# ScottHCL/recommend

Measured on AMD Instinct MI355X. Metric: ranked samples/sec (fwd+bwd) at B=4096 seq=128; AUC parity vs ref, higher is better.
Workload: dtype f32-emulated (fp16-pair / split-bf16); 1 GPU; C2: OneTrans 4L d128 H4 f512 L_NS12 L_S128 (seq 3x42), Criteo-shape 13 dense + 26 ids, replicated tables, fwd+bwd+optimizer; global_batch=4096, per_gpu_batch=4096, seq_len=128, parallelism=dp1

## Files before the change

### include/onetrans_hip.h

```cpp
#ifndef ONETRANS_HIP_H
#define ONETRANS_HIP_H

#include <stddef.h>
#include <stdint.h>

#ifdef __cplusplus
extern "C" {
#endif

#define OT_OK 0
#define OT_ERR_INVALID_ARG 1
#define OT_ERR_UNSUPPORTED 2
#define OT_ERR_HIP 3

#define OT_GEMM_NN 0
#define OT_GEMM_NT 1

#define OT_AX_NONE 0
#define OT_AX_RMSNORM 1
#define OT_AX_GELU 2
#define OT_AX_BF16 4
#define OT_AX_BF16_RMSNORM 5

#define OT_EPI_BIAS 1
// ... 9 lines not shown
#define OT_EPI_AUX_BF16 1024
#define OT_WG_D_BF16 8
#define OT_WG_D_KEEPBITS 16

int ot_version(void);
const char* ot_get_last_error_string(void);

int ot_gemm_tile_rows(void);
#define OT_MATMUL_F32 0
#define OT_MATMUL_SPLIT_BF16 1
#define OT_MATMUL_BF16 2
int ot_mixed_gemm(int mode, const float* A, int64_t lda, int K, const int32_t* in_rows,
                  int a_xform, const float* a_rstd, const float* a_gamma,
                  const float* W, int64_t w_gstride, int64_t ldw, int N,
                  const int32_t* tile_group, int ntiles,
                  const float* bias, int64_t bias_gstride,
                  float* C, int64_t ldc, const int32_t* out_rows, int epi,
                  const float* res, int64_t ldres, int res_tok,
                  const float* aux, int64_t ldaux,
                  uint32_t seed, uint32_t site, float drop_rate, int tail_K, int tail_I,
                  const int32_t* tail_pos, int precision, void* stream);
typedef struct ot_rms_epilogue {
  size_t struct_size;
  float* rstd_out; float eps;
  const float* x; int64_t ldx;
  const float* gamma; const float* rstd;
  const float* dres; int64_t lddres;
  int dres_tail_K, dres_tail_I;
  const int32_t* dres_tail_inv;
  float* dx_masked; int64_t lddxm;
  float* dgamma; int accumulate_dgamma;
  void* workspace; size_t ws_bytes;
  float* rowdot; int rowdot_n;
  uint16_t* gelu_out; int64_t ldgelu;
  uint16_t* xn_out; int64_t ldxn;
  uint16_t* c16_out; int64_t ldc16;
  float* rowmax_out; int rowmax_n;
  const float* a_rowmax; int a_rowmax_n;
  float* amax_out;
  float* rowabs_out; int rowabs_n;
} ot_rms_epilogue;
size_t ot_mixed_gemm_rms_workspace_size(int ntiles, int N);
int ot_mixed_gemm_rms(int mode, const float* A, int64_t lda, int K, const int32_t* in_rows,
                      int a_xform, const float* a_rstd, const float* a_gamma,
                      const float* W, int64_t w_gstride, int64_t ldw, int N,
                      const int32_t* tile_group, int ntiles,
                      const float* bias, int64_t bias_gstride,
                      float* C, int64_t ldc, const int32_t* out_rows, int epi,
                      const float* res, int64_t ldres, int res_tok,
                      const float* aux, int64_t ldaux,
                      uint32_t seed, uint32_t site, float drop_rate, int tail_K, int tail_I,
                      const int32_t* tail_pos, const ot_rms_epilogue* rms, int precision, void* stream);

size_t ot_wgrad_workspace_size(int nchunks, int K, int N);
int ot_mixed_gemm_wgrad(const float* A, int64_t lda, const int32_t* a_rows, int a_xform,
                        const float* a_rstd, const float* a_gamma,
                        const float* D, int64_t ldd, const int32_t* d_rows, int K, int N,
                        const int32_t* chunks, int nchunks, const int32_t* gchunk, int ngroups,
                        float* dW, int64_t dw_gstride, float* db, int64_t db_gstride,
                        int accumulate, void* workspace, size_t ws_bytes, int precision, void* stream);

int ot_mixed_gemm_wgrad_ex(const float* A, int64_t lda, const int32_t* a_rows, int a_xform,
                           const float* a_rstd, const float* a_gamma,
                           const float* D, int64_t ldd, const int32_t* d_rows, int K, int N,
                           const int32_t* chunks, int nchunks, const int32_t* gchunk, int ngroups,
                           float* dW, int64_t dw_gstride, float* db, int64_t db_gstride,
                           int accumulate, void* workspace, size_t ws_bytes, const float* a_bound,
                           const float* d_bound, int precision, void* stream);

int ot_mixed_gemm_wgrad_keep(const float* A, int64_t lda, const int32_t* a_rows, int a_xform,
                             const float* D, int64_t ldd, const int32_t* d_rows, int K, int N,
                             const int32_t* chunks, int nchunks, const int32_t* gchunk, int ngroups,
                             float* dW, int64_t dw_gstride, float* db, int64_t db_gstride,
                             int accumulate, void* workspace, size_t ws_bytes, const float* a_bound,
                             const float* d_bound, const uint32_t* keep, int64_t ldkeep, float d_scale,
                             int precision, void* stream);

int ot_transpose_banks(const float* src, float* dst, const int64_t* banks_dev, int nbanks, int64_t total_tiles,
                       void* stream);

size_t ot_split_image_elems(int G, int N, int K);
int ot_split_images(const float* base, const int64_t* desc_dev, int ndesc, int64_t total_units, uint16_t* img,
                    int precision, void* stream);
int ot_mixed_gemm_img(int mode, const float* A, int64_t lda, int K, const int32_t* in_rows,
                      int a_xform, const float* a_rstd, const float* a_gamma,
                      const float* W, int64_t w_gstride, int64_t ldw, int N,
                      const int32_t* tile_group, int ntiles,
                      const float* bias, int64_t bias_gstride,
                      float* C, int64_t ldc, const int32_t* out_rows, int epi,
                      const float* res, int64_t ldres, int res_tok,
                      const float* aux, int64_t ldaux,
                      uint32_t seed, uint32_t site, float drop_rate, int tail_K, int tail_I,
                      const int32_t* tail_pos, const uint16_t* b_image, int image_ntn, int image_tn0,
                      int precision, void* stream);
int ot_plane_wide(int on);
int ot_wgrad_wide(int on);
int ot_plane_rowmeta(int on);
int ot_plane_panel(int on);
int ot_plane_panel_launches(void);
int ot_mixed_gemm_rms_img(int mode, const float* A, int64_t lda, int K, const int32_t* in_rows,
                          int a_xform, const float* a_rstd, const float* a_gamma,
                          const float* W, int64_t w_gstride, int64_t ldw, int N,
                          const int32_t* tile_group, int ntiles,
                          const float* bias, int64_t bias_gstride,
                          float* C, int64_t ldc, const int32_t* out_rows, int epi,
                          const float* res, int64_t ldres, int res_tok,
                          const float* aux, int64_t ldaux,
                          uint32_t seed, uint32_t site, float drop_rate, int tail_K, int tail_I,
                          const int32_t* tail_pos, const ot_rms_epilogue* rms, const uint16_t* b_image,
                          int image_ntn, int image_tn0, int precision, void* stream);

typedef struct ot_ffn_fused_args {
  size_t struct_size;
  const float* x1; int64_t ldx1;
  const int32_t* rows;
  const int32_t* tile_group; int ntiles;
  const float* rstd;
  const uint16_t* w1_image; int w1_groups;
  const uint16_t* w2_image; int w2_groups;
  const float* b1; int64_t b1_gstride;
  const float* b2; int64_t b2_gstride;
  int f;
  float* u_out; int64_t ldu;
  float* u_amax;
  float* x2; int64_t ldx2;
  float* rstd_out; float eps;
  uint32_t seed, site; float drop_rate;
  int tail_K, tail_I; const int32_t* tail_pos;
} ot_ffn_fused_args;
int ot_ffn_fused_fwd(const ot_ffn_fused_args* args, void* stream);
int ot_ffn_fused(int on);

typedef struct ot_ffn_fused_bwd_args {
  size_t struct_size;
  const float* dy2; int64_t lddy2;
  const float* dy2_rowmax; int dy2_rowmax_n;
  const int32_t* rows;
  const int32_t* tile_group; int ntiles;
  const uint16_t* w2_image; int w2_groups;
  const uint16_t* w1_image; int w1_groups;
  int f;
  const float* u; int64_t ldu;
  float* du; int64_t lddu;
  float* du_amax;
  const float* x1; int64_t ldx1;
  const float* gamma; const float* rstd;
  const float* dres; int64_t lddres;
  float* dx1; int64_t lddx1;
  float* dx_masked; int64_t lddxm;
  float* dgamma; int accumulate_dgamma;
  void* workspace; size_t ws_bytes;
  float* amax_out; float* rowabs_out; int rowabs_n;
  uint32_t seed, site; float drop_rate;
  int tail_K, tail_I; const int32_t* tail_pos;
} ot_ffn_fused_bwd_args;
int ot_ffn_fused_bwd(const ot_ffn_fused_bwd_args* args, void* stream);
int ot_ffn_fused_bwd_on(int on);
int ot_ffn_fused_bwd_mask(const ot_ffn_fused_bwd_args* args, uint32_t mask_site, uint32_t* keep_out, int64_t ldkeep,
                          void* stream);
int ot_bwd_mask_fused(int on);

int ot_attn_fwd(const float* qkv, int64_t ld, int B, int H, int I, int K, const int32_t* qpos,
                int head_dim, float* out, float* lse, int precision, void* stream);
size_t ot_attn_fwd_fp8_workspace_size(int B, int H, int I, int head_dim);
int ot_attn_fwd_fp8(const float* qkv, int64_t ld, int B, int H, int I, int K, const int32_t* qpos,
                    int head_dim, float* out, float* lse, void* workspace, size_t ws_bytes, void* stream);
// ... 274 lines not shown
```

### recommend_amd/_lib.py

```python

from __future__ import annotations

import ctypes
import os
from ctypes import c_float, c_int, c_int64, c_size_t, c_uint32, c_void_p, c_char_p

_HERE = os.path.dirname(os.path.abspath(__file__))
LIB_PATH = os.environ.get('ONETRANS_HIP_LIB') or os.path.join(_HERE, 'libonetrans_hip.so')
HEADER = os.path.join(os.path.dirname(_HERE), 'include', 'onetrans_hip.h')

OT_GEMM_NN, OT_GEMM_NT = 0, 1
OT_AX_NONE, OT_AX_RMSNORM, OT_AX_GELU, OT_AX_BF16, OT_AX_BF16_RMSNORM = 0, 1, 2, 4, 5
OT_EPI_BIAS, OT_EPI_GELU_BWD, OT_EPI_GELU = 1, 2, 4
OT_EPI_DROPOUT, OT_EPI_RESIDUAL, OT_EPI_ACCUMULATE = 8, 16, 32
OT_EPI_ROW_RSTD, OT_EPI_RMSNORM_BWD, OT_EPI_ROWDOT = 64, 128, 256
OT_EPI_C_BF16 = 512
OT_EPI_AUX_BF16 = 1024
OT_ATTN_DQKV_BF16 = 1
OT_ATTN_QKV_BF16 = 2
OT_ATTN_DQ_PART_BF16 = 4
OT_WG_D_BF16 = 8
OT_WG_D_KEEPBITS = 16
OT_MATMUL_F32, OT_MATMUL_SPLIT_BF16, OT_MATMUL_BF16 = 0, 1, 2
OT_FP8_DEQUANT, OT_FP8_TWO_TERM = 1, 2
# ... 28 lines not shown
                ('tile_group', c_void_p), ('ntiles', c_int), ('rstd', c_void_p),
                ('w1_image', c_void_p), ('w1_groups', c_int), ('w2_image', c_void_p), ('w2_groups', c_int),
                ('b1', c_void_p), ('b1_gstride', c_int64), ('b2', c_void_p), ('b2_gstride', c_int64),
                ('f', c_int), ('u_out', c_void_p), ('ldu', c_int64), ('u_amax', c_void_p),
                ('x2', c_void_p), ('ldx2', c_int64), ('rstd_out', c_void_p), ('eps', c_float),
                ('seed', c_uint32), ('site', c_uint32), ('drop_rate', c_float),
                ('tail_K', c_int), ('tail_I', c_int), ('tail_pos', c_void_p)]


class FfnFusedBwdArgs(ctypes.Structure):
    _fields_ = [('struct_size', c_size_t), ('dy2', c_void_p), ('lddy2', c_int64),
                ('dy2_rowmax', c_void_p), ('dy2_rowmax_n', c_int), ('rows', c_void_p),
                ('tile_group', c_void_p), ('ntiles', c_int),
                ('w2_image', c_void_p), ('w2_groups', c_int), ('w1_image', c_void_p), ('w1_groups', c_int),
                ('f', c_int), ('u', c_void_p), ('ldu', c_int64), ('du', c_void_p), ('lddu', c_int64),
                ('du_amax', c_void_p), ('x1', c_void_p), ('ldx1', c_int64), ('gamma', c_void_p), ('rstd', c_void_p),
                ('dres', c_void_p), ('lddres', c_int64), ('dx1', c_void_p), ('lddx1', c_int64),
                ('dx_masked', c_void_p), ('lddxm', c_int64), ('dgamma', c_void_p), ('accumulate_dgamma', c_int),
                ('workspace', c_void_p), ('ws_bytes', c_size_t),
                ('amax_out', c_void_p), ('rowabs_out', c_void_p), ('rowabs_n', c_int),
                ('seed', c_uint32), ('site', c_uint32), ('drop_rate', c_float),
                ('tail_K', c_int), ('tail_I', c_int), ('tail_pos', c_void_p)]


class SeqTime(ctypes.Structure):
    _fields_ = [('times', c_void_p), ('stride_b', c_int64), ('L', ctypes.c_int32), ('map_off', ctypes.c_int32)]


class NsBag(ctypes.Structure):
    _fields_ = [('table', c_void_p), ('ids', c_void_p), ('weights', c_void_p), ('row_offset', c_int64),
                ('num_rows', c_int64), ('ids_stride', c_int64), ('weights_stride', c_int64),
                ('width', ctypes.c_int32), ('cap', ctypes.c_int32), ('col', ctypes.c_int32),
                ('pooling', ctypes.c_int32)]


OT_BAG_SUM, OT_BAG_MEAN = 0, 1
BAG_POOLINGS = {'sum': OT_BAG_SUM, 'mean': OT_BAG_MEAN}
NS_BAG_MAX = 32
NS_BAG_MAX_WIDTH = 256
SEQ_TIME_MAX_L = 4096
SEQ_TIME_MAX_SEQ = 32

P = c_void_p
I64 = c_int64

SIGNATURES = {
    'ot_version': (c_int, []),
    'ot_get_last_error_string': (c_char_p, []),
    'ot_gemm_tile_rows': (c_int, []),
    'ot_mixed_gemm': (c_int, [c_int, P, I64, c_int, P, c_int, P, P, P, I64, I64, c_int, P, c_int, P, I64,
                              P, I64, P, c_int, P, I64, c_int, P, I64, c_uint32, c_uint32, c_float, c_int,
                              c_int, P, c_int, P]),
    'ot_mixed_gemm_rms_workspace_size': (c_size_t, [c_int, c_int]),
    'ot_mixed_gemm_rms': (c_int, [c_int, P, I64, c_int, P, c_int, P, P, P, I64, I64, c_int, P, c_int, P, I64,
                                  P, I64, P, c_int, P, I64, c_int, P, I64, c_uint32, c_uint32, c_float, c_int,
                                  c_int, P, P, c_int, P]),
    'ot_wgrad_workspace_size': (c_size_t, [c_int, c_int, c_int]),
    'ot_mixed_gemm_wgrad': (c_int, [P, I64, P, c_int, P, P, P, I64, P, c_int, c_int, P, c_int, P, c_int, P,
                                    I64, P, I64, c_int, P, c_size_t, c_int, P]),
    'ot_mixed_gemm_wgrad_ex': (c_int, [P, I64, P, c_int, P, P, P, I64, P, c_int, c_int, P, c_int, P, c_int, P,
                                       I64, P, I64, c_int, P, c_size_t, P, P, c_int, P]),
    'ot_mixed_gemm_wgrad_keep': (c_int, [P, I64, P, c_int, P, I64, P, c_int, c_int, P, c_int, P, c_int, P, I64, P,
                                         I64, c_int, P, c_size_t, P, P, P, I64, c_float, c_int, P]),
    'ot_transpose_banks': (c_int, [P, P, P, c_int, I64, P]),
    'ot_mixed_gemm_img': (c_int, [c_int, P, I64, c_int, P, c_int, P, P, P, I64, I64, c_int, P, c_int, P, I64,
                                  P, I64, P, c_int, P, I64, c_int, P, I64, c_uint32, c_uint32, c_float, c_int,
                                  c_int, P, P, c_int, c_int, c_int, P]),
    'ot_mixed_gemm_rms_img': (c_int, [c_int, P, I64, c_int, P, c_int, P, P, P, I64, I64, c_int, P, c_int, P, I64,
                                      P, I64, P, c_int, P, I64, c_int, P, I64, c_uint32, c_uint32, c_float, c_int,
                                      c_int, P, P, P, c_int, c_int, c_int, P]),
    'ot_split_image_elems': (c_size_t, [c_int, c_int, c_int]),
    'ot_plane_wide': (c_int, [c_int]),
    'ot_wgrad_wide': (c_int, [c_int]),
    'ot_plane_rowmeta': (c_int, [c_int]),
    'ot_plane_panel': (c_int, [c_int]),
    'ot_plane_panel_launches': (c_int, []),
    'ot_ffn_fused_fwd': (c_int, [P, P]),
    'ot_ffn_fused': (c_int, [c_int]),
    'ot_ffn_fused_bwd': (c_int, [P, P]),
    'ot_ffn_fused_bwd_on': (c_int, [c_int]),
    'ot_ffn_fused_bwd_mask': (c_int, [P, c_uint32, P, I64, P]),
    'ot_bwd_mask_fused': (c_int, [c_int]),
    'ot_split_images': (c_int, [P, P, c_int, I64, P, c_int, P]),
    'ot_attn_fwd': (c_int, [P, I64, c_int, c_int, c_int, c_int, P, c_int, P, P, c_int, P]),
    'ot_attn_fwd_fp8_workspace_size': (c_size_t, [c_int, c_int, c_int, c_int]),
    'ot_attn_fwd_fp8': (c_int, [P, I64, c_int, c_int, c_int, c_int, P, c_int, P, P, P, c_size_t, P]),
    'ot_attn_fwd_fp8_ex': (c_int, [P, I64, c_int, c_int, c_int, c_int, P, c_int, P, P, P, c_size_t, c_int, P]),
    'ot_attn_fwd_fp8_deq16': (c_int, [P, I64, c_int, c_int, c_int, c_int, P, c_int, P, P, P, c_size_t, c_int, P, P]),
    'ot_attn_bwd_workspace_size': (c_size_t, [c_int, c_int, c_int]),
    'ot_attn_bwd': (c_int, [P, I64, P, P, P, c_int, c_int, c_int, c_int, P, c_int, P, P, c_int, P]),
    'ot_attn_bwd_ex_workspace_size': (c_size_t, [c_int, c_int, c_int, c_int, c_int, c_int, c_int]),
    'ot_attn_bwd_ex': (c_int, [P, I64, P, P, P, c_int, c_int, c_int, c_int, P, c_int, P, P, c_size_t, c_int, P]),
    'ot_attn_bwd_dqkv_bf16_supported': (c_int, [c_int, c_int, c_int, c_int, c_int]),
    'ot_attn_bwd_bf16_forms': (c_int, [c_int, c_int, c_int, c_int, c_int]),
    'ot_attn_slice_supported': (c_int, [c_int, c_int, c_int, c_int]),
    'ot_attn_bwd_flags_workspace_size': (c_size_t, [c_int, c_int, c_int, c_int, c_int, c_int, c_int, c_int]),
    'ot_attn_bwd_flags': (c_int, [P, I64, P, P, P, c_int, c_int, c_int, c_int, P, c_int, P, c_int, P, c_size_t, c_int, P]),
    'ot_attn_fwd_cached': (c_int, [P, I64, P, I64, P, c_int, c_int, c_int, c_int, c_int, c_int, P, P]),
    'ot_attn_fwd_cached_lse': (c_int, [P, I64, P, I64, P, c_int, c_int, c_int, c_int, c_int, c_int, P, P, P]),
    'ot_attn_bwd_cached_workspace_size': (c_size_t, [c_int, c_int, c_int, c_int, c_int, c_int, c_int]),
    'ot_attn_bwd_cached': (c_int, [P, I64, P, I64, P, c_int, c_int, c_int, c_int, c_int, c_int, c_int, P, P, P, P, P,
                                   c_int, P, c_size_t, P]),
    'ot_attn_amax_supported': (c_int, [c_int, c_int, c_int, c_int, c_int]),
    'ot_attn_fwd_amax': (c_int, [P, I64, c_int, c_int, c_int, c_int, P, c_int, P, P, P, P, c_int, P]),
    'ot_attn_bwd_amax': (c_int, [P, I64, P, P, P, c_int, c_int, c_int, c_int, P, c_int, P, P, c_size_t, P, P, c_int,
                                 P]),
    'ot_pyramid_select': (c_int, [P, c_float, c_int, c_int, c_int, c_int, P, P, P, c_int, P]),
    'ot_rmsnorm_fwd': (c_int, [P, I64, P, P, I64, P, I64, c_int, c_float, P]),
    'ot_rmsnorm_bwd_workspace_size': (c_size_t, [I64, c_int]),
    'ot_rmsnorm_bwd': (c_int, [P, I64, P, I64, P, P, P, I64, c_int, c_int, P, P, I64, P, I64, c_uint32,
                               c_uint32, c_float, c_int, c_int, P, P, c_int, I64, c_int, P, c_size_t, P]),
    'ot_dropout_apply': (c_int, [P, I64, P, I64, I64, c_int, c_uint32, c_uint32, c_float, c_int, c_int, P, P]),
    'ot_dropout_apply_bf16': (c_int, [P, I64, P, I64, I64, c_int, c_uint32, c_uint32, c_float, c_int, c_int, P, P]),
    'ot_rows_absmax': (c_int, [P, I64, I64, c_int, P, c_int, P]),
    'ot_dropout_rowmax_supported': (c_int, [c_int]),
    'ot_dropout_apply_ex': (c_int, [P, I64, P, I64, I64, c_int, c_uint32, c_uint32, c_float, c_int, c_int, P, P, P,
                                    c_int, P]),
    'ot_rows_colsum_workspace_size': (c_size_t, [I64, c_int]),
    'ot_rows_colsum': (c_int, [P, I64, P, I64, c_int, P, c_int, P, c_size_t, P]),
    'ot_ns_assemble': (c_int, [P, c_int, P, c_int, P, I64, P]),
    'ot_ns_grad_pack': (c_int, [P, c_int, c_int, P, I64, c_int, P, P, P]),
    'ot_fill_rows': (c_int, [P, I64, P, I64, P, c_int, P]),
    'ot_seq_rows': (c_int, [P, I64, c_int, c_int, I64, P, P]),
    'ot_head_fwd': (c_int, [P, P, P, c_int, c_int, c_int, P, P, P]),
    'ot_head_bwd_workspace_size': (c_size_t, [c_int, c_int, c_int]),
    'ot_head_bwd': (c_int, [P, P, P, P, c_int, c_int, c_int, P, P, P, I64, I64, c_int, P, c_size_t, P]),
    'ot_bce_workspace_size': (c_size_t, [c_int, c_int]),
    'ot_bce_fwd': (c_int, [P, P, c_int, c_int, P, P, c_size_t, P]),
    'ot_bce_bwd': (c_int, [P, P, P, c_int, c_int, P, P]),
    'ot_task_loss_fwd': (c_int, [P, P, c_int, c_int, c_uint32, P, P, c_size_t, P]),
    'ot_task_loss_bwd': (c_int, [P, P, P, c_int, c_int, c_uint32, P, P]),
    'ot_task_loss_logits_fwd': (c_int, [P, P, P, c_int, c_int, c_uint32, P, P, c_size_t, P]),
    'ot_task_loss_logits_bwd': (c_int, [P, P, P, c_int, c_int, c_uint32, P, P]),
    'ot_task_loss_weighted_workspace_size': (c_size_t, [c_int, c_int]),
    'ot_task_loss_weighted_fwd': (c_int, [P, P, P, P, I64, P, c_int, c_int, c_uint32, c_int, P, P, P, c_size_t, P]),
    'ot_task_loss_weighted_bwd': (c_int, [P, P, P, I64, P, P, P, c_int, c_int, c_uint32, c_int, P, P]),
    'ot_head_bwd_ex': (c_int, [P, P, P, P, P, c_int, c_int, c_int, P, P, P, I64, I64, c_int, P, c_size_t, P]),
    'ot_sparse_adagrad_workspace_size': (c_size_t, [I64, c_int]),
    'ot_sparse_adagrad': (c_int, [P, P, c_int, I64, P, P, I64, c_float, c_float, c_float, P, c_size_t, P]),
    'ot_sparse_grad_dense': (c_int, [c_int, I64, P, P, I64, P, P, c_size_t, P]),
    'ot_dense_adagrad_workspace_size': (c_size_t, []),
    'ot_dense_adagrad': (c_int, [P, P, P, I64, c_int, c_float, c_float, c_float, P, c_size_t, P]),
    'ot_sparse_prepare': (c_int, [c_int, I64, P, P, I64, P, P, c_size_t, P]),
    'ot_sparse_finish': (c_int, [P, P, c_int, I64, c_float, c_float, c_float, P, P, c_size_t, P]),
    'ot_sparse_adagrad_rowwise': (c_int, [P, P, c_int, I64, P, P, I64, c_float, c_float, c_float, P, c_size_t, P]),
    'ot_dense_adagrad_rowwise': (c_int, [P, P, P, I64, c_int, c_float, c_float, c_float, P, c_size_t, P]),
    'ot_sparse_finish_rowwise': (c_int, [P, P, c_int, I64, c_float, c_float, c_float, P, P, c_size_t, P]),
    'ot_shard_route_workspace_size': (c_size_t, [I64]),
    'ot_shard_route': (c_int, [P, I64, I64, c_int, P, P, P, P, c_size_t, P]),
    'ot_shard_route_unique_workspace_size': (c_size_t, [I64]),
    'ot_shard_route_unique': (c_int, [P, I64, I64, c_int, P, P, P, P, P, P, c_size_t, P]),
    'ot_segment_rows_sum': (c_int, [P, P, P, I64, c_int, P, P]),
    'ot_segment_rows_sum_workspace_size': (c_size_t, [I64, I64, c_int]),
    'ot_segment_rows_sum_ex': (c_int, [P, P, P, I64, I64, c_int, P, P, c_size_t, P]),
    'ot_gather_rows': (c_int, [P, c_int, P, I64, P, P]),
    'ot_permute_rows': (c_int, [P, P, I64, c_int, c_int, P, P]),
    'ot_hash_uniform_rows': (c_int, [P, I64, c_int, c_int, c_int, c_uint32, c_float, c_float, P]),
    'ot_clip_rmsprop_workspace_size': (c_size_t, [c_int, I64]),
    'ot_clip_rmsprop': (c_int, [P, P, P, P, P, c_int, I64, c_float, c_float, c_float, c_float, c_float, P,
                                c_size_t, P]),
    'ot_clip_adam_workspace_size': (c_size_t, [c_int, I64]),
    'ot_clip_adam': (c_int, [P, P, P, P, P, c_int, I64, c_float, c_float, c_float, c_float, I64, c_float, P,
                             c_size_t, P]),
    'ot_metrics_workspace_size': (c_size_t, [c_int, c_int]),
    'ot_metrics_update': (c_int, [P, P, c_int, c_int, I64, P, c_int, P, P, P, c_size_t, P]),
    'ot_metrics_weighted_workspace_size': (c_size_t, [c_int, c_int]),
# ... 78 lines not shown
```

### recommend_amd/csrc/gemm_images.hip

```cpp
#include "gemm.h"

namespace ot {

__device__ __forceinline__ const int64_t* image_unit(const int64_t* desc, int nd, int64_t unit, int64_t& g, int64_t& tn,
                                                     int64_t& ks) {
  int b = 0;
  while (b + 1 < nd && desc[10 * (b + 1) + 6] <= unit) ++b;
  const int64_t* d = desc + 10 * b;
  const int64_t G = d[7], N = d[8], K = d[9];
  const int64_t ntn = (N + GT - 1) / GT, nks = K / 16;
  int64_t u = unit - d[6];
  if (u >= G * ntn * nks) return nullptr;
  g = u / (ntn * nks);
  u %= ntn * nks;
  tn = u / nks;
  ks = u % nks;
  return d;
}

__global__ __launch_bounds__(256) void image_colscale_kernel(const float* __restrict__ base, const int64_t* __restrict__ desc,
                                                             int nd, uint16_t* img) {
  int64_t g, tn, ks;
  const int64_t* d = image_unit(desc, nd, blockIdx.x, g, tn, ks);
  if (!d || ks != 0 || d[4] == -1) return;
  const int64_t N = d[8], K = d[9];
  const int n = threadIdx.x >> 1, hh = threadIdx.x & 1;
  const int64_t gn = tn * GT + n;
  float m = 0.f;
  if (gn < N) {
    const float* src = base + d[0] + g * d[3] + gn * d[1];
#pragma unroll 8
    for (int64_t k = hh; k < K; k += 2) {
      float x = src[k * d[2]];
      if (d[4] >= 0) x *= base[d[4] + k];
      m = fmaxf(m, fabsf(x));
    }
  }
  m = fmaxf(m, __shfl_xor(m, 1, 64));
  float* csc = reinterpret_cast<float*>(img + d[5] + ((int64_t)blockIdx.x - d[6]) * (PG_B_BYTES / 2) + 2 * GT * 16);
  if (hh == 0) csc[n] = pow2_scale14(m);
  if (threadIdx.x == 0) reinterpret_cast<uint32_t*>(csc)[GT] = PAIR_IMAGE_TAG;
}

__global__ __launch_bounds__(256) void split_images_kernel(const float* __restrict__ base, const int64_t* __restrict__ desc,
                                                           int nd, uint16_t* img, int one) {
  const int64_t unit = blockIdx.x;
  int64_t g, tn, ks;
  const int64_t* d = image_unit(desc, nd, unit, g, tn, ks);
  if (!d) return;
  const int64_t N = d[8];
  const int n = threadIdx.x >> 1, hh = threadIdx.x & 1;
  const int64_t gn = tn * GT + n;
  const float* src = base + d[0] + g * d[3] + gn * d[1];
  float v[8];
#pragma unroll
  for (int j = 0; j < 8; ++j) {
    const int64_t k = ks * 16 + 8 * hh + j;
    float x = gn < N ? src[k * d[2]] : 0.f;
    if (d[4] >= 0) x *= base[d[4] + k];
    v[j] = x;
  }
  uint16_t* dst = img + d[5] + (unit - d[6]) * (PG_B_BYTES / 2);
  u32x4 pl[3];
  const bool pair = !one && d[4] != -1;
  if (one) {
    split8t<1>(v, pl);
  } else if (pair) {
    const float sn = reinterpret_cast<const float*>(dst - ks * (PG_B_BYTES / 2) + 2 * GT * 16)[n];
    pair8(v, sn, pl);
  } else {
    split8(v, pl);
  }
  const int npl = one ? 1 : pair ? 2 : 3;
#pragma unroll
  for (int q = 0; q < 3; ++q)
    if (q < npl) *reinterpret_cast<u32x4*>(dst + q * GT * 16 + n * 16 + 8 * (hh ^ ((n >> 3) & 1))) = pl[q];
}

}

using namespace ot;

extern "C" size_t ot_split_image_elems(int G, int N, int K) {
  if (G <= 0 || N <= 0 || K <= 0 || K % 16) return 0;
  return (size_t)G * ceil_div(N, GT) * (K / 16) * (PG_B_BYTES / 2);
}

extern "C" int ot_split_images(const float* base, const int64_t* desc_dev, int ndesc, int64_t total_units,
                               uint16_t* img, int precision, void* stream) {
  OT_REQUIRE(base && desc_dev && img && ndesc > 0 && total_units >= 0, "ot_split_images: bad args");
  OT_REQUIRE(precision == OT_MATMUL_SPLIT_BF16 || precision == OT_MATMUL_BF16,
             "ot_split_images: precision %d has no plane images", precision);
  if (total_units == 0) return OT_OK;
  if (precision == OT_MATMUL_SPLIT_BF16) {
    hipLaunchKernelGGL(image_colscale_kernel, dim3((unsigned)total_units), dim3(256), 0, (hipStream_t)stream, base,
                       desc_dev, ndesc, img);
    OT_LAUNCH_CHECK("ot_split_images(column scales)");
  }
  hipLaunchKernelGGL(split_images_kernel, dim3((unsigned)total_units), dim3(256), 0, (hipStream_t)stream, base,
                     desc_dev, ndesc, img, precision == OT_MATMUL_BF16 ? 1 : 0);
  OT_LAUNCH_CHECK("ot_split_images");
  return OT_OK;
}
```

### recommend_amd/kernels.py

```python

from __future__ import annotations

import contextlib
import ctypes
import functools
import os
import threading
from typing import Optional, Tuple, Union

import torch

from . import _lib
from ._lib import call, size

Ptrish = Union[None, torch.Tensor, Tuple[torch.Tensor, int]]


class Probe:

    def __init__(self):
        self.recs = []

    def begin(self):
        ev = torch.cuda.Event(enable_timing=True)
# ... 272 lines not shown

def plane_wide(on: int = -1) -> int:
    return _lib.size('ot_plane_wide', int(on))


def wgrad_wide(on: int = -1) -> int:
    return _lib.size('ot_wgrad_wide', int(on))


def plane_rowmeta(on: int = -1) -> int:
    return _lib.size('ot_plane_rowmeta', int(on))


def plane_panel(on: int = -1) -> int:
    return _lib.size('ot_plane_panel', int(on))


def plane_panel_launches() -> int:
    return _lib.size('ot_plane_panel_launches')


def ffn_fused(on: int = -1) -> int:
    return _lib.size('ot_ffn_fused', int(on))


FFN_FUSED_MAX_F = 1024


def ffn_fused_fwd(x1: Ptrish, ldx1: int, rows: Ptrish, tile_group: Ptrish, ntiles: int, rstd: Ptrish, w1_image,
                  w1_groups: int, w2_image, w2_groups: int, b1: Ptrish, b1_gstride: int, b2: Ptrish, b2_gstride: int,
                  f: int, x2: Ptrish, ldx2: int, *, u_out: Ptrish = None, ldu: int = 0, u_amax: Ptrish = None,
                  rstd_out: Ptrish = None, eps: float = 1e-6, seed: int = 0, site: int = 0, drop: float = 0.0,
                  tail: Tuple[int, int] = (1, 1), m_rows: int = 0) -> None:
    a = _lib.FfnFusedArgs(ctypes.sizeof(_lib.FfnFusedArgs), ptr(x1), ldx1, ptr(rows), ptr(tile_group), ntiles,
                          ptr(rstd), ptr(w1_image), int(w1_groups), ptr(w2_image), int(w2_groups), ptr(b1),
                          b1_gstride, ptr(b2), b2_gstride, f, ptr(u_out), ldu, ptr(u_amax), ptr(x2), ldx2,
                          ptr(rstd_out), float(eps), seed & 0xFFFFFFFF, site, float(drop), tail[0], tail[1],
                          _sel(tail))
    ev = _probe.begin() if _probe is not None else None
    call('ot_ffn_fused_fwd', ctypes.byref(a), stream())
    if ev is not None:
        M = m_rows or ntiles * 128
        _probe.end('mixed_gemm', 2.0 * M * 128 * f * 2, ev, f'ffn_fused M{M} f{f} u{int(u_out is not None)}',
                   4.0 * M * 128 * 3 + 4.0 * M * f * (u_out is not None)
                   + 4.0 * M * (1 + (rstd_out is not None)), 3)


def ffn_fused_bwd_on(on: int = -1) -> int:
    return _lib.size('ot_ffn_fused_bwd_on', int(on))


def bwd_mask_fused(on: int = -1) -> int:
    return _lib.size('ot_bwd_mask_fused', int(on))


def ffn_fused_bwd(dy2: Ptrish, lddy2: int, dy2_rowmax: Ptrish, dy2_rowmax_n: int, rows: Ptrish, tile_group: Ptrish,
                  ntiles: int, w2_image, w2_groups: int, w1_image, w1_groups: int, f: int, u: Ptrish, ldu: int,
                  du: Ptrish, lddu: int, x1: Ptrish, ldx1: int, gamma: Ptrish, rstd: Ptrish, dx1: Ptrish, lddx1: int,
                  dgamma: Ptrish, *, du_amax: Ptrish = None, dres: Ptrish = None, lddres: int = 0,
                  dx_masked: Ptrish = None, lddxm: int = 0, accumulate_dgamma: bool = False, amax_out: Ptrish = None,
                  rowabs_out: Ptrish = None, rowabs_n: int = 0, seed: int = 0, site: int = 0, drop: float = 0.0,
                  tail: Tuple[int, int] = (1, 1), m_rows: int = 0, device=None, mask_site: Optional[int] = None,
                  keep_out: Ptrish = None, ldkeep: int = 4) -> None:
    ws = workspace(size('ot_mixed_gemm_rms_workspace_size', ntiles, 128),
                   device if device is not None else (dx1[0] if isinstance(dx1, tuple) else dx1).device)
    a = _lib.FfnFusedBwdArgs(ctypes.sizeof(_lib.FfnFusedBwdArgs), ptr(dy2), lddy2, ptr(dy2_rowmax), int(dy2_rowmax_n),
                             ptr(rows), ptr(tile_group), ntiles, ptr(w2_image), int(w2_groups), ptr(w1_image),
                             int(w1_groups), f, ptr(u), ldu, ptr(du), lddu, ptr(du_amax), ptr(x1), ldx1, ptr(gamma),
                             ptr(rstd), ptr(dres), lddres, ptr(dx1), lddx1, ptr(dx_masked), lddxm, ptr(dgamma),
                             int(accumulate_dgamma), ptr(ws), ws.numel(), ptr(amax_out), ptr(rowabs_out),
                             int(rowabs_n), seed & 0xFFFFFFFF, site, float(drop), tail[0], tail[1], _sel(tail))
    ev = _probe.begin() if _probe is not None else None
    if mask_site is not None:
        call('ot_ffn_fused_bwd_mask', ctypes.byref(a), mask_site, ptr(keep_out), ldkeep, stream())
    else:
        call('ot_ffn_fused_bwd', ctypes.byref(a), stream())
    if ev is not None:
        M = m_rows or ntiles * 128
        _probe.end('mixed_gemm', 2.0 * M * 128 * f * 2, ev, f'ffn_fused_bwd M{M} f{f} drop{int(drop > 0)}',
                   4.0 * M * 128 * (3 + (dres is not None) + (dx_masked is not None)) + 4.0 * M * f * 2
                   + 4.0 * M * (1 + dy2_rowmax_n), 3)


def split_images(base, desc_dev, ndesc, total_units, img) -> None:
    call('ot_split_images', ptr(base), ptr(desc_dev), ndesc, total_units, ptr(img), _prec(), stream())


def attn_fwd(qkv: torch.Tensor, ld: int, B: int, H: int, I: int, K: int, hd: int, out: torch.Tensor,
             lse: torch.Tensor, qpos: Optional[torch.Tensor] = None, fp8: bool = False,
             dequant: bool = False, fp8_terms: int = 1, deq16: Optional[torch.Tensor] = None,
             amax: Optional[torch.Tensor] = None, rowmax: Optional[torch.Tensor] = None) -> None:
    if fp8 and fp8_terms not in (1, 2):
        raise ValueError(f'fp8_terms {fp8_terms}: 1 or 2')
    ws = None
    if fp8:
        ws = workspace(size('ot_attn_fwd_fp8_workspace_size', B, H, I, hd), qkv.device)
    ev = _probe.begin() if _probe is not None else None
    if fp8 and deq16 is not None:
        call('ot_attn_fwd_fp8_deq16', ptr(qkv), ld, B, H, I, K, ptr(qpos), hd, ptr(out), ptr(lse), ptr(ws),
             ws.numel(), _lib.OT_FP8_TWO_TERM if fp8_terms == 2 else 0, ptr(deq16), stream())
    elif fp8:
        call('ot_attn_fwd_fp8_ex', ptr(qkv), ld, B, H, I, K, ptr(qpos), hd, ptr(out), ptr(lse), ptr(ws),
             ws.numel(), (_lib.OT_FP8_DEQUANT if dequant else 0) | (_lib.OT_FP8_TWO_TERM if fp8_terms == 2 else 0),
             stream())
    elif amax is not None or rowmax is not None:
        call('ot_attn_fwd_amax', ptr(qkv), ld, B, H, I, K, ptr(qpos), hd, ptr(out), ptr(lse), ptr(amax), ptr(rowmax),
             _prec(), stream())
    else:
        call('ot_attn_fwd', ptr(qkv), ld, B, H, I, K, ptr(qpos), hd, ptr(out), ptr(lse), _prec(), stream())
    if ev is not None:
        _probe.end('attention', 4.0 * (K * I - K * (K - 1) / 2) * hd * H * B, ev,
                   f'fwd{"_fp8" if fp8 else ""} I{I} K{K} hd{hd}')


def attn_bwd_bf16_forms(I, K, hd, qpos=None) -> int:
    return int(_lib.load().ot_attn_bwd_bf16_forms(I, K, hd, int(qpos is not None), _prec()))


def attn_bwd_bf16_supported(I, K, hd, qpos=None) -> bool:
    return bool(_lib.load().ot_attn_bwd_dqkv_bf16_supported(I, K, hd, int(qpos is not None), _prec()))


def attn_amax_supported(I, K, hd, qpos=None, backward: bool = False) -> bool:
    return bool(_lib.load().ot_attn_amax_supported(I, K, hd, int(qpos is not None), _prec()) & (2 if backward else 1))


def attn_bwd(qkv, ld, out, dout, lse, B, H, I, K, hd, dqkv, qpos=None, dq_part_bf16: bool = False,
             amax=None, rowmax=None) -> None:
    flags = ((_lib.OT_ATTN_DQKV_BF16 if dqkv.dtype == torch.int16 else 0)
             | (_lib.OT_ATTN_QKV_BF16 if qkv.dtype == torch.int16 else 0)
             | (_lib.OT_ATTN_DQ_PART_BF16 if dq_part_bf16 and dqkv.dtype == torch.int16
                and attn_bwd_bf16_forms(I, K, hd, qpos) & _lib.OT_ATTN_DQ_PART_BF16 else 0))
    ws = workspace(size('ot_attn_bwd_flags_workspace_size', B, H, I, K, hd, int(qpos is not None), flags, _prec()),
                   qkv.device)
    ev = _probe.begin() if _probe is not None else None
    if amax is not None or rowmax is not None:
        call('ot_attn_bwd_amax', ptr(qkv), ld, ptr(out), ptr(dout), ptr(lse), B, H, I, K, ptr(qpos), hd, ptr(dqkv),
             ptr(ws), ws.numel(), ptr(amax), ptr(rowmax), _prec(), stream())
    else:
        call('ot_attn_bwd_flags', ptr(qkv), ld, ptr(out), ptr(dout), ptr(lse), B, H, I, K, ptr(qpos), hd,
             ptr(dqkv), flags, ptr(ws), ws.numel(), _prec(), stream())
    if ev is not None:
        _probe.end('attention', 8.0 * (K * I - K * (K - 1) / 2) * hd * H * B, ev, f'bwd I{I} K{K} hd{hd}')


def last_fold(on: int = -1) -> int:
    return _lib.size('ot_last_fold', int(on))


def attn_fold_supported(d: int, H: int) -> bool:
    return bool(_lib.size('ot_attn_fold_supported', int(d), int(H)))


def attn_fold_rows(I: int, ded0: int, ded1: int) -> int:
    return _lib.size('ot_attn_fold_rows', int(I), int(ded0), int(ded1))


def _fold_common(x, ldx, rstd, gamma, w, ldw, wT, ldwT, qkv, ldqkv, B, H, I, hd, ded):
    return (ptr(x), ldx, ptr(rstd), ptr(gamma), ptr(w), ldw, ptr(wT), ldwT, ptr(qkv), ldqkv, B, H, I, hd, ded[0],
            ded[1])


def attn_fold_fwd(x, ldx, rstd, gamma, w, ldw, wT, ldwT, qkv, ldqkv, B, H, I, hd, ded, o, lse, y) -> None:
    ev = _probe.begin() if _probe is not None else None
    call('ot_attn_fold_fwd', *_fold_common(x, ldx, rstd, gamma, w, ldw, wT, ldwT, qkv, ldqkv, B, H, I, hd, ded),
         ptr(o), ptr(lse), ptr(y), stream())
# ... 517 lines not shown
```

Measured before the change: 214,400 samples/s.

## Fuse weight image column-scale and split into one persistent tile kernel

Replaces the two-kernel weight-image build (a column-scale pass, then a per-unit split pass) with one persistent kernel. Each block walks whole N-tiles, computes the column max scale, and then writes all K-step split planes for that tile, using vectorized loads when strides allow. The grid is capped at three blocks per CU and the kernel is on by default behind an env/API toggle. The aim is to cut a launch and redundant per-unit work on the weight-preparation step each iteration, at the cost of less parallelism per tile.

```diff
diff --git a/include/onetrans_hip.h b/include/onetrans_hip.h
--- a/include/onetrans_hip.h
+++ b/include/onetrans_hip.h
@@ -115,6 +115,7 @@
 size_t ot_split_image_elems(int G, int N, int K);
 int ot_split_images(const float* base, const int64_t* desc_dev, int ndesc, int64_t total_units, uint16_t* img,
                     int precision, void* stream);
+int ot_image_build(int on);
 int ot_mixed_gemm_img(int mode, const float* A, int64_t lda, int K, const int32_t* in_rows,
                       int a_xform, const float* a_rstd, const float* a_gamma,
                       const float* W, int64_t w_gstride, int64_t ldw, int N,
diff --git a/recommend_amd/_lib.py b/recommend_amd/_lib.py
--- a/recommend_amd/_lib.py
+++ b/recommend_amd/_lib.py
@@ -134,6 +134,7 @@
     'ot_ffn_fused_bwd_mask': (c_int, [P, c_uint32, P, I64, P]),
     'ot_bwd_mask_fused': (c_int, [c_int]),
     'ot_split_images': (c_int, [P, P, c_int, I64, P, c_int, P]),
+    'ot_image_build': (c_int, [c_int]),
     'ot_attn_fwd': (c_int, [P, I64, c_int, c_int, c_int, c_int, P, c_int, P, P, c_int, P]),
     'ot_attn_fwd_fp8_workspace_size': (c_size_t, [c_int, c_int, c_int, c_int]),
     'ot_attn_fwd_fp8': (c_int, [P, I64, c_int, c_int, c_int, c_int, P, c_int, P, P, P, c_size_t, P]),
diff --git a/recommend_amd/csrc/gemm_images.hip b/recommend_amd/csrc/gemm_images.hip
--- a/recommend_amd/csrc/gemm_images.hip
+++ b/recommend_amd/csrc/gemm_images.hip
@@ -1,3 +1,6 @@
+#include <atomic>
+#include <cstdlib>
+
 #include "gemm.h"
 
 namespace ot {
@@ -77,9 +80,185 @@
     if (q < npl) *reinterpret_cast<u32x4*>(dst + q * GT * 16 + n * 16 + 8 * (hh ^ ((n >> 3) & 1))) = pl[q];
 }
 
+constexpr int IMG_MAXD = 256;
+constexpr int IMG_GRID_PER_CU = 3;
+
+template <bool VK>
+__device__ __forceinline__ void image_load8(const float* __restrict__ row, bool live, int64_t sk,
+                                            const float* __restrict__ ksc, int64_t k0, float (&v)[8]) {
+  if constexpr (VK) {
+    f32x4 a = {0.f, 0.f, 0.f, 0.f}, b = a;
+    if (live) {
+      a = *reinterpret_cast<const f32x4*>(row + k0);
+      b = *reinterpret_cast<const f32x4*>(row + k0 + 4);
+    }
+    if (ksc) {
+      a *= *reinterpret_cast<const f32x4*>(ksc + k0);
+      b *= *reinterpret_cast<const f32x4*>(ksc + k0 + 4);
+    }
+#pragma unroll
+    for (int j = 0; j < 4; ++j) v[j] = a[j], v[4 + j] = b[j];
+  } else {
+#pragma unroll
+    for (int j = 0; j < 8; ++j) {
+      float x = live ? row[(k0 + j) * sk] : 0.f;
+      if (ksc) x *= ksc[k0 + j];
+      v[j] = x;
+    }
+  }
+}
+
+template <bool VK>
+__device__ __forceinline__ float image_colmax(const float* __restrict__ row, bool live, int64_t sk,
+                                              const float* __restrict__ ksc, int hh, int nks) {
+  float m = 0.f;
+  if (live) {
+#pragma unroll 4
+    for (int ks = 0; ks < nks; ++ks) {
+      float v[8];
+      image_load8<VK>(row, true, sk, ksc, ks * 16 + 8 * hh, v);
+#pragma unroll
+      for (int j = 0; j < 8; ++j) m = fmaxf(m, fabsf(v[j]));
+    }
+  }
+  return fmaxf(m, __shfl_xor(m, 1, 64));
+}
+
+template <bool VK>
+__device__ __forceinline__ void image_split_units(const float* __restrict__ row, bool live, int64_t sk,
+                                                  const float* __restrict__ ksc, int n, int hh, int nks, int form,
+                                                  float scale, uint16_t* dst) {
+  uint16_t* out = dst + n * 16 + 8 * (hh ^ ((n >> 3) & 1));
+#pragma unroll 2
+  for (int ks = 0; ks < nks; ++ks, out += PG_B_BYTES / 2) {
+    float v[8];
+    image_load8<VK>(row, live, sk, ksc, ks * 16 + 8 * hh, v);
+    u32x4 pl[3];
+    if (form == 1) {
+      split8t<1>(v, pl);
+      *reinterpret_cast<u32x4*>(out) = pl[0];
+    } else if (form == 2) {
+      pair8(v, scale, pl);
+      *reinterpret_cast<u32x4*>(out) = pl[0];
+      *reinterpret_cast<u32x4*>(out + GT * 16) = pl[1];
+    } else {
+      split8(v, pl);
+#pragma unroll
+      for (int q = 0; q < 3; ++q) *reinterpret_cast<u32x4*>(out + q * GT * 16) = pl[q];
+    }
+  }
+}
+
+__global__ __launch_bounds__(256) void build_images_kernel(const float* __restrict__ base, const int64_t* __restrict__ desc,
+                                                           int nd, int64_t total_units, uint16_t* img, int one) {
+  __shared__ int tiles[IMG_MAXD];
+  __shared__ float part[8][GT];
+  const int tid = threadIdx.x;
+  {
+    int c = 0;
+    if (tid < nd) c = (int)(desc[10 * tid + 7] * ((desc[10 * tid + 8] + GT - 1) / GT));
+    tiles[tid] = c;
+    __syncthreads();
+    for (int o = 1; o < IMG_MAXD; o <<= 1) {
+      const int a = tid >= o ? tiles[tid - o] : 0;
+      __syncthreads();
+      tiles[tid] += a;
+      __syncthreads();
+    }
+  }
+  const int ntiles = tiles[IMG_MAXD - 1];
+  const int n = tid >> 1, hh = tid & 1;
+  for (int t = blockIdx.x; t < ntiles; t += gridDim.x) {
+    int lo = 0, hi = nd - 1;
+    while (lo < hi) {
+      const int mid = (lo + hi) >> 1;
+      if (tiles[mid] > t) hi = mid; else lo = mid + 1;
+    }
+    const int64_t* d = desc + 10 * lo;
+    const int64_t sn = d[1], sk = d[2], kso = d[4], N = d[8], K = d[9];
+    const int ntn = (int)((N + GT - 1) / GT), nks_all = (int)(K / 16);
+    const int local = t - (lo ? tiles[lo - 1] : 0), g = local / ntn, tn = local % ntn;
+    const int64_t u0 = (int64_t)local * nks_all;
+    const int64_t left = total_units - (d[6] + u0);
+    if (left <= 0) continue;
+    const int nks = left < nks_all ? (int)left : nks_all;
+    const int64_t so = d[0] + g * d[3];
+    const float* src = base + so;
+    const float* ksc = kso >= 0 ? base + kso : nullptr;
+    const int form = one ? 1 : kso != -1 ? 2 : 0;
+    uint16_t* dst = img + d[5] + u0 * (PG_B_BYTES / 2);
+    const int64_t gn = (int64_t)tn * GT + n;
+    const bool live = gn < N;
+    const float* row = src + gn * sn;
+    const bool al = (reinterpret_cast<uintptr_t>(base) & 15) == 0 && (so & 3) == 0;
+    const bool vk = al && sk == 1 && (sn & 3) == 0 && (kso < 0 || (kso & 3) == 0);
+    const bool vn = al && sn == 1 && (sk & 3) == 0 && (N & 3) == 0;
+    float scale = 1.f;
+    if (form == 2) {
+      float m;
+      if (vk) {
+        m = image_colmax<true>(row, live, sk, ksc, hh, nks_all);
+      } else if (vn) {
+        const int r = tid >> 5, c = tid & 31;
+        f32x4 m4 = {0.f, 0.f, 0.f, 0.f};
+        if ((int64_t)tn * GT + 4 * c < N) {
+          const float* p = src + (int64_t)tn * GT + 4 * c;
+#pragma unroll 4
+          for (int64_t k = r; k < K; k += 8) {
+            f32x4 x = *reinterpret_cast<const f32x4*>(p + k * sk);
+            if (ksc) x *= ksc[k];
+#pragma unroll
+            for (int j = 0; j < 4; ++j) m4[j] = fmaxf(m4[j], fabsf(x[j]));
+          }
+        }
+        *reinterpret_cast<f32x4*>(&part[r][4 * c]) = m4;
+        __syncthreads();
+        m = part[0][n];
+#pragma unroll
+        for (int q = 1; q < 8; ++q) m = fmaxf(m, part[q][n]);
+        __syncthreads();
+      } else {
+        m = image_colmax<false>(row, live, sk, ksc, hh, nks_all);
+      }
+      scale = pow2_scale14(m);
+      float* csc = reinterpret_cast<float*>(dst + 2 * GT * 16);
+      if (hh == 0) csc[n] = scale;
+      if (tid == 0) reinterpret_cast<uint32_t*>(csc)[GT] = PAIR_IMAGE_TAG;
+    }
+    if (vk) image_split_units<true>(row, live, sk, ksc, n, hh, nks, form, scale, dst);
+    else image_split_units<false>(row, live, sk, ksc, n, hh, nks, form, scale, dst);
+  }
+}
+
+#ifndef OT_IMAGE_BUILD
+#define OT_IMAGE_BUILD 1
+#endif
+static int image_build_initial() {
+  const char* e = getenv("ONETRANS_IMAGE_BUILD");
+  return e && *e ? (atoi(e) != 0) : OT_IMAGE_BUILD;
+}
+static std::atomic<int> g_image_build{image_build_initial()};
+
+static int image_grid_cap() {
+  static const int cap = [] {
+    int dev = 0, cus = 0;
+    if (hipGetDevice(&dev) != hipSuccess ||
+        hipDeviceGetAttribute(&cus, hipDeviceAttributeMultiprocessorCount, dev) != hipSuccess || cus <= 0)
+      cus = 256;
+    return IMG_GRID_PER_CU * cus;
+  }();
+  return cap;
+}
+
 }
 
 using namespace ot;
+
+extern "C" int ot_image_build(int on) {
+  const int old = g_image_build.load(std::memory_order_relaxed);
+  if (on >= 0) g_image_build.store(on ? 1 : 0, std::memory_order_relaxed);
+  return old;
+}
 
 extern "C" size_t ot_split_image_elems(int G, int N, int K) {
   if (G <= 0 || N <= 0 || K <= 0 || K % 16) return 0;
@@ -92,6 +271,14 @@
   OT_REQUIRE(precision == OT_MATMUL_SPLIT_BF16 || precision == OT_MATMUL_BF16,
              "ot_split_images: precision %d has no plane images", precision);
   if (total_units == 0) return OT_OK;
+  OT_REQUIRE(total_units <= 0x7fffffff, "ot_split_images: %lld units", (long long)total_units);
+  if (g_image_build.load(std::memory_order_relaxed) && ndesc <= IMG_MAXD) {
+    const int64_t cap = image_grid_cap();
+    hipLaunchKernelGGL(build_images_kernel, dim3((unsigned)(total_units < cap ? total_units : cap)), dim3(256), 0,
+                       (hipStream_t)stream, base, desc_dev, ndesc, total_units, img, precision == OT_MATMUL_BF16 ? 1 : 0);
+    OT_LAUNCH_CHECK("ot_split_images(build)");
+    return OT_OK;
+  }
   if (precision == OT_MATMUL_SPLIT_BF16) {
     hipLaunchKernelGGL(image_colscale_kernel, dim3((unsigned)total_units), dim3(256), 0, (hipStream_t)stream, base,
                        desc_dev, ndesc, img);
diff --git a/recommend_amd/kernels.py b/recommend_amd/kernels.py
--- a/recommend_amd/kernels.py
+++ b/recommend_amd/kernels.py
@@ -378,6 +378,10 @@
                    + 4.0 * M * (1 + dy2_rowmax_n), 3)
 
 
+def image_build(on: int = -1) -> int:
+    return _lib.size('ot_image_build', int(on))
+
+
 def split_images(base, desc_dev, ndesc, total_units, img) -> None:
     call('ot_split_images', ptr(base), ptr(desc_dev), ndesc, total_units, ptr(img), _prec(), stream())
 
```

Measured after the change: 219,800 samples/s, median of 6. +2.5%, better.
